# pierregab/VUB_Image_denoising

Measured on AMD Instinct MI355X. Metric: images/sec (256x256x3) RDUNet diffusion train step, higher is better.
Workload: dtype bf16; 1 GPU; RDUNet_T(base_filters=32) diffusion train step, fwd+Charbonnier+bwd+clip+AdamW; global_batch=16, per_gpu_batch=16, parallelism=dp1, optimizer_step=every step, launcher=single process

## Files before the change

### vub_image_denoising_amd/csrc/conv3_big.hip

```cpp
#include "conv3_tile.h"

#include <cstdlib>

namespace {

__device__ __attribute__((aligned(64))) unsigned int g_big_zero[16];


template <int N>
__device__ __forceinline__ void wait_vm() { asm volatile("s_waitcnt vmcnt(%0)" ::"n"(N) : "memory"); }

__device__ __forceinline__ void glds16(const void* src, unsigned dst) {
  unsigned keep;
  asm volatile("s_mov_b32 %0, m0\n\ts_mov_b32 m0, %2\n\ts_nop 0\n\tglobal_load_lds_dwordx4 %1, off\n\ts_mov_b32 m0, %0"
               : "=&s"(keep)
               : "v"(src), "s"(__builtin_amdgcn_readfirstlane(dst))
               : "memory");
}
__device__ __forceinline__ unsigned lds_addr(const unsigned char* p) {
  return (unsigned)(uintptr_t)(const __attribute__((address_space(3))) unsigned char*)p;
}

constexpr int TWB = 16;
constexpr int RS = TWB + 2;
constexpr int LDS_CAP = 160 * 1024;
constexpr int COL_MAX = 640;

enum { EP_FWD = 0, EP_FWD_RES = 1, EP_PLAIN = 2, EP_ACC = 3, EP_RES = 4 };

template <int CK>
__device__ __forceinline__ int hswz(int u, int x) {
  return CK == 64 ? (u ^ (x & 7)) : (u ^ ((x >> 1) & 3));
}

template <int TH, int BN, int WM, int CK, int NW = 8>
struct PtCfg {
  static constexpr int NTB = 64 * NW;
  static constexpr int BPC = NW == 8 ? 1 : 2;
  static constexpr int BM = TH * TWB;
  static constexpr int HWP = (TH + 2) * RS;
  static constexpr int RB = CK * 2;
  static constexpr int H_PIECES = (HWP * RB + 1023) / 1024;
  static constexpr int HALO_BYTES = H_PIECES * 1024;
  static constexpr int KC = (9 * CK + 63) / 64 * 64;
  static constexpr int SPC = KC / 64;
  static constexpr int SS = (SPC + 1) / 2;
  static constexpr int RW = 256;
  static constexpr int W_BYTES = BN * RW;
  static constexpr int W_PIECES = W_BYTES / 1024;
  static constexpr int W_PW = (W_PIECES + NW - 1) / NW;
  static constexpr int TAB = 2 * COL_MAX * 4;
  static constexpr int LDS = 2 * HALO_BYTES + 2 * W_BYTES + TAB;
  static constexpr int WN = NW / WM;
  static constexpr int WTM = BM / WM, WTN = BN / WN;
  static constexpr int MT = WTM / 16, NTL = WTN / 16;
  static constexpr bool OK = BPC * LDS <= LDS_CAP && MT >= 1 && NTL >= 1 && WTM % 16 == 0 && WTN % 16 == 0 &&
                             (CK == 32 || CK == 64) && WM * WN == NW && (NW == 8 || NW == 4);
};

template <int NLO, int NHI, int SPLIT>
__device__ __forceinline__ void wait_split(int wave) {
  if (wave < SPLIT) wait_vm<NHI>();
  else wait_vm<NLO>();
}

template <int TH, int BN, int WM, int CK, int EP, bool GO, int NW = 8>
__global__ __launch_bounds__(64 * NW, 2) void conv3_big_kernel(rdn_conv_desc d, int tiles_x, int tiles_y, int nitems) {
  using Cfg = PtCfg<TH, BN, WM, CK, NW>;
  constexpr int NTB = Cfg::NTB;
  constexpr int RB = Cfg::RB, RW = Cfg::RW, SPC = Cfg::SPC, SS = Cfg::SS;
  constexpr int WTN = Cfg::WTN, MT = Cfg::MT, NTL = Cfg::NTL, W_PW = Cfg::W_PW, HP = Cfg::H_PIECES;
  constexpr bool FWD = EP == EP_FWD || EP == EP_FWD_RES;
  constexpr bool RES = EP == EP_FWD_RES || EP == EP_RES;
  constexpr bool ACC = EP == EP_ACC;
  constexpr bool GOK = GO && !FWD;
  constexpr bool W16 = !GOK && MT % 2 == 0;
  static_assert(Cfg::OK, "conv3_big geometry");

  __shared__ __attribute__((aligned(1024))) unsigned char lds[Cfg::LDS];
  unsigned char* const halo = lds;
  unsigned char* const wst = lds + 2 * Cfg::HALO_BYTES;
  float* const tab = (float*)(wst + 2 * Cfg::W_BYTES);

  const int tid = threadIdx.x, lane = tid & 63, wave = tid >> 6;
  const int wm = wave % WM, wn = wave / WM;
  const int r = lane & 15, g = lane >> 4;
  const int ncb = d.ncols / BN;
  const int H = d.h, W = d.w;
  const int nch = d.cin / CK;

  const int per = gridDim.x >> 3, xcd = blockIdx.x & 7;
  const int it_lo = (int)((int64_t)nitems * xcd / 8), it_hi = (int)((int64_t)nitems * (xcd + 1) / 8);
  int item = it_lo + (blockIdx.x >> 3);

  const bool spre = (d.flags & RDN_EPI_STORE_PRE) != 0;
  if constexpr (FWD) {
    for (int c = tid; c < d.ncols; c += NTB) {
      tab[c] = d.bias[c];
      tab[COL_MAX + c] = d.alpha[c];
    }
  }
  if constexpr (GOK) {
    for (int c = tid; c < d.ncols - d.gout_c0; c += NTB) tab[COL_MAX + c] = d.gout_alpha[c];
  }

  struct Geo { int nimg, y0, x0, n0; };
  auto geo = [&](int itm) {
    Geo q;
    const int cb = itm % ncb;
    int t = itm / ncb;
    const int tx = t % tiles_x;
    t /= tiles_x;
    q.y0 = (t % tiles_y) * TH;
    q.x0 = tx * TWB;
    q.nimg = t / tiles_y;
    q.n0 = cb * BN;
    return q;
  };

  auto issue_h = [&](const Geo& q, int c, int hb) {
    const unsigned dst = lds_addr(halo) + hb * Cfg::HALO_BYTES;
    const bf16* const xb = (const bf16*)d.x + (((int64_t)q.nimg * H + (q.y0 - 1)) * W + (q.x0 - 1)) * d.x_ps;
#pragma unroll
    for (int k = 0; k < (HP + NW - 1) / NW; ++k) {
      const int pc = wave + NW * k;
      if (pc >= HP) break;
      const int off = pc * 1024 + lane * 16;
      const int hp = off / RB, pu = (off % RB) / 16;
      const int hy = hp / RS, hx = hp - (hp / RS) * RS;
      const int u = hswz<CK>(pu, hx);
      const bool ok =
          hp < Cfg::HWP && (unsigned)(q.y0 - 1 + hy) < (unsigned)H && (unsigned)(q.x0 - 1 + hx) < (unsigned)W;
      const void* src = ok ? (const void*)(xb + (int64_t)(hy * W + hx) * d.x_ps +
                                           rdn_coff32(d.x_c0 + c * CK + u * 8, (int)d.x_ps, (int)d.x_pl))
                           : (const void*)g_big_zero;
      glds16(src, dst + pc * 1024);
    }
  };
  auto issue_w = [&](int n0, int c, int jj, int wb) {
    const unsigned dst = lds_addr(wst) + wb * Cfg::W_BYTES;
#pragma unroll
    for (int k = 0; k < W_PW; ++k) {
      const int pc = wave + NW * k;
      if (pc >= Cfg::W_PIECES) break;
      const int row = 4 * pc + (lane >> 4);
      const int u = (lane & 15) ^ (row & 15);
      const bool ok = 2 * jj + 1 < SPC || u < 8;
      const void* src = ok ? (const void*)((const bf16*)d.wp + (int64_t)(n0 + row) * d.kp + c * Cfg::KC + jj * 128 +
                                           u * 8)
                           : (const void*)g_big_zero;
      glds16(src, dst + pc * 1024);
    }
  };

  int a_off[CK == 64 ? 6 : 3];
#pragma unroll
  for (int ks = 0; ks < (CK == 64 ? 2 : 1); ++ks)
#pragma unroll
    for (int dx = 0; dx < 3; ++dx) a_off[ks * 3 + dx] = (r + dx) * RB + hswz<CK>(ks * 4 + g, r + dx) * 16;
  const int a_row0 = (wm * MT) * RS * RB;
  const int b_lane = (wn * WTN + r) * RW;
  int b_off[4];
#pragma unroll
  for (int hk = 0; hk < 4; ++hk) b_off[hk] = ((hk * 4 + g) ^ r) * 16;

  f32x4 acc[MT][NTL];
  auto zero_acc = [&]() {
#pragma unroll
    for (int i = 0; i < MT; ++i)
#pragma unroll
      for (int jn = 0; jn < NTL; ++jn) acc[i][jn] = f32x4{0.f, 0.f, 0.f, 0.f};
  };

  auto compute_pf = [&](int jj, const unsigned char* ph, const unsigned char* pbs) {
    auto valid = [&](int q) { return 2 * jj + (q >> 1) < SPC && (2 * jj + (q >> 1)) * 64 + (q & 1) * 32 < 9 * CK; };
    u32x4 af[2][MT], bfr[2][NTL];
    auto rd = [&](int q, int buf) {
#ifdef BIG_DIAG_NO_LDS
#pragma unroll
      for (int i = 0; i < MT; ++i) asm volatile("" : "=v"(af[buf][i]));
#pragma unroll
      for (int jn = 0; jn < NTL; ++jn) asm volatile("" : "=v"(bfr[buf][jn]));
      return;
#endif
      const int k0 = (2 * jj + (q >> 1)) * 64 + (q & 1) * 32;
      const int tap = k0 / CK, ksub = (k0 - tap * CK) / 32;
      const int dy = tap / 3, dx = tap % 3;
      const unsigned char* pa = ph + a_row0 + dy * RS * RB + a_off[ksub * 3 + dx];
#pragma unroll
      for (int i = 0; i < MT; ++i) af[buf][i] = *(const u32x4*)(pa + i * RS * RB);
#pragma unroll
      for (int jn = 0; jn < NTL; ++jn) bfr[buf][jn] = *(const u32x4*)(pbs + jn * 16 * RW + b_off[q]);
    };
    rd(0, 0);
#pragma unroll
    for (int q = 0; q < 4; ++q) {
      if (!valid(q)) break;
      if (q + 1 < 4 && valid(q + 1)) rd(q + 1, (q + 1) & 1);
      __builtin_amdgcn_sched_barrier(0);
#ifdef BIG_DIAG_NO_MFMA
#pragma unroll
      for (int i = 0; i < MT; ++i) asm volatile("" ::"v"(af[q & 1][i]));
#pragma unroll
      for (int jn = 0; jn < NTL; ++jn) asm volatile("" ::"v"(bfr[q & 1][jn]));
      continue;
#endif
#pragma unroll
      for (int i = 0; i < MT; ++i)
#pragma unroll
        for (int jn = 0; jn < NTL; ++jn)
          acc[i][jn] = __builtin_amdgcn_mfma_f32_16x16x32_bf16(__builtin_bit_cast(bf16x8, bfr[q & 1][jn]),
                                                               __builtin_bit_cast(bf16x8, af[q & 1][i]), acc[i][jn], 0,
                                                               0, 0);
    }
  };
  auto compute_roll = [&](int jj, const unsigned char* ph, const unsigned char* pbs) {
    auto valid = [&](int q) { return 2 * jj + (q >> 1) < SPC && (2 * jj + (q >> 1)) * 64 + (q & 1) * 32 < 9 * CK; };
    u32x4 af[MT], bfr[2][NTL];
    auto pa_of = [&](int q) {
      const int k0 = (2 * jj + (q >> 1)) * 64 + (q & 1) * 32;
      const int tap = k0 / CK, ksub = (k0 - tap * CK) / 32;
      const int dy = tap / 3, dx = tap % 3;
      return ph + a_row0 + dy * RS * RB + a_off[ksub * 3 + dx];
    };
    auto rdb = [&](int q, int buf) {
#pragma unroll
      for (int jn = 0; jn < NTL; ++jn) bfr[buf][jn] = *(const u32x4*)(pbs + jn * 16 * RW + b_off[q]);
    };
    {
      const unsigned char* pa = pa_of(0);
#pragma unroll
      for (int i = 0; i < MT; ++i) af[i] = *(const u32x4*)(pa + i * RS * RB);
      rdb(0, 0);
    }
#pragma unroll
    for (int q = 0; q < 4; ++q) {
      if (!valid(q)) break;
      const bool nx = q + 1 < 4 && valid(q + 1);
      if (nx) rdb(q + 1, (q + 1) & 1);
      const unsigned char* pn = pa_of(nx ? q + 1 : q);
#pragma unroll
      for (int i = 0; i < MT; ++i) {
        __builtin_amdgcn_sched_barrier(0);
#pragma unroll
        for (int jn = 0; jn < NTL; ++jn)
          acc[i][jn] = __builtin_amdgcn_mfma_f32_16x16x32_bf16(__builtin_bit_cast(bf16x8, bfr[q & 1][jn]),
                                                               __builtin_bit_cast(bf16x8, af[i]), acc[i][jn], 0, 0, 0);
        __builtin_amdgcn_sched_barrier(0);
        if (nx) af[i] = *(const u32x4*)(pn + i * RS * RB);
      }
    }
  };
  auto compute_np = [&](int jj, const unsigned char* ph, const unsigned char* pbs) {
#pragma unroll
    for (int h = 0; h < 2; ++h) {
      const int j = 2 * jj + h;
      if (j >= SPC) break;
#pragma unroll
      for (int ks = 0; ks < 2; ++ks) {
        const int k0 = j * 64 + ks * 32;
        if (k0 >= 9 * CK) break;
        const int tap = k0 / CK, ksub = (k0 - tap * CK) / 32;
        const int dy = tap / 3, dx = tap % 3;
        const unsigned char* pa = ph + a_row0 + dy * RS * RB + a_off[ksub * 3 + dx];
        __builtin_amdgcn_sched_barrier(0);
        u32x4 af[MT], bfr[NTL];
#pragma unroll
        for (int i = 0; i < MT; ++i) af[i] = *(const u32x4*)(pa + i * RS * RB);
#pragma unroll
        for (int jn = 0; jn < NTL; ++jn) bfr[jn] = *(const u32x4*)(pbs + jn * 16 * RW + b_off[2 * h + ks]);
#pragma unroll
        for (int i = 0; i < MT; ++i)
#pragma unroll
          for (int jn = 0; jn < NTL; ++jn)
            acc[i][jn] = __builtin_amdgcn_mfma_f32_16x16x32_bf16(__builtin_bit_cast(bf16x8, bfr[jn]),
                                                                 __builtin_bit_cast(bf16x8, af[i]), acc[i][jn], 0, 0,
                                                                 0);
      }
    }
  };
  constexpr bool ROLL = BN == 128 && CK == 64 && (GOK || EP == EP_FWD_RES);
  constexpr bool NOPF = BN == 128 && CK == 64 && GOK && EP == EP_RES;
  auto compute = [&](int jj, const unsigned char* ph, const unsigned char* pbs) {
    if constexpr (NOPF) compute_np(jj, ph, pbs);
    else if constexpr (ROLL) compute_roll(jj, ph, pbs);
    else compute_pf(jj, ph, pbs);
  };

  u32x2 eop[(RES || ACC) ? MT : 1][(RES || ACC) ? NTL : 1];
  u32x2 gpre[GOK ? MT : 1][GOK ? NTL : 1];
  auto epi_load = [&](const Geo& q) {
    const int64_t pix0 = ((int64_t)q.nimg * H + q.y0) * W + q.x0;
    const bool col_ok = q.x0 + r < W;
    if constexpr ((RES || ACC) && W16) {
      const int ops = (int)d.out_ps;
      const int eps = RES ? (int)d.res_ps : ops;
      const __amdgpu_buffer_rsrc_t re =
          rdn_rsrc(RES ? (const bf16*)d.res + pix0 * d.res_ps : (const bf16*)d.out + pix0 * d.out_ps);
#pragma unroll
      for (int jn = 0; jn < NTL; ++jn) {
        const int cl = q.n0 + wn * WTN + jn * 16 + 8 * (g >> 1);
        const int coff =
            RES ? rdn_coff32(d.res_c0 + cl, eps, (int)d.res_pl) : rdn_coff32(d.out_c0 + cl, ops, (int)d.out_pl);
        const bool cok = col_ok & (RES ? cl < d.res_climit : true);
#pragma unroll
        for (int p = 0; p < MT / 2; ++p) {
          const int i = 2 * p + (g & 1);
          const bool ok = cok & (q.y0 + wm * MT + i < H);
          const u32x4 u = rdn_ld16(re, ok, (((wm * MT + i) * W + r) * eps + coff) * 2);
          eop[2 * p][jn] = u32x2{u[0], u[1]};
          eop[2 * p + 1][jn] = u32x2{u[2], u[3]};
        }
      }
    } else if constexpr (RES || ACC) {
      const int ops = (int)d.out_ps;
      const int eps = RES ? (int)d.res_ps : ops;
      const __amdgpu_buffer_rsrc_t re =
          rdn_rsrc(RES ? (const bf16*)d.res + pix0 * d.res_ps : (const bf16*)d.out + pix0 * d.out_ps);
#pragma unroll
      for (int jn = 0; jn < NTL; ++jn) {
        const int cl = q.n0 + wn * WTN + jn * 16 + g * 4;
        const int coff =
            RES ? rdn_coff32(d.res_c0 + cl, eps, (int)d.res_pl) : rdn_coff32(d.out_c0 + cl, ops, (int)d.out_pl);
        const bool cok = col_ok & (RES ? cl < d.res_climit : true);
#pragma unroll
        for (int i = 0; i < MT; ++i) {
          const bool ok = cok & (q.y0 + wm * MT + i < H);
          eop[i][jn] = rdn_ld8(re, ok, (((wm * MT + i) * W + r) * eps + coff) * 2);
        }
      }
    }
    if constexpr (GOK) {
      const __amdgpu_buffer_rsrc_t rg = rdn_rsrc((const bf16*)d.gout_pre + pix0 * d.gout_pre_ps);
      const int gps = (int)d.gout_pre_ps;
#pragma unroll
      for (int jn = 0; jn < NTL; ++jn) {
        const int cl = q.n0 + wn * WTN + jn * 16 + g * 4;
        const bool gok = col_ok & (cl >= d.gout_c0);
#pragma unroll
        for (int i = 0; i < MT; ++i)
          gpre[i][jn] = rdn_ld8(rg, gok & (q.y0 + wm * MT + i < H), (((wm * MT + i) * W + r) * gps + cl - d.gout_c0) * 2);
      }
    }
  };
  auto epilogue16 = [&](const Geo& q) {
    epi_load(q);
    const int64_t pix0 = ((int64_t)q.nimg * H + q.y0) * W + q.x0;
    const __amdgpu_buffer_rsrc_t ro = rdn_rsrc((const bf16*)d.out + pix0 * d.out_ps);
    const int ops = (int)d.out_ps, pps = (int)d.pre_ps;
    const bool col_ok = q.x0 + r < W;
    const __amdgpu_buffer_rsrc_t rp = FWD && spre ? rdn_rsrc((const bf16*)d.pre + pix0 * d.pre_ps) : ro;
#pragma unroll
    for (int jn = 0; jn < NTL; ++jn) {
      const int cl = q.n0 + wn * WTN + jn * 16 + 8 * (g >> 1);
      f32x4 b0 = {0.f, 0.f, 0.f, 0.f}, b1 = b0, a0 = b0, a1 = b0;
      if constexpr (FWD) {
        b0 = *(const f32x4*)(tab + cl);
        b1 = *(const f32x4*)(tab + cl + 4);
        a0 = *(const f32x4*)(tab + COL_MAX + cl);
        a1 = *(const f32x4*)(tab + COL_MAX + cl + 4);
      }
      const int co = rdn_coff32(d.out_c0 + cl, ops, (int)d.out_pl);
      const int cp = FWD ? rdn_coff32(cl, pps, (int)d.pre_pl) : 0;
      const bool res_ok = RES ? cl < d.res_climit : true;
#pragma unroll
      for (int p = 0; p < MT / 2; ++p) {
        const int i = 2 * p + (g & 1);
        const bool ok = col_ok & (q.y0 + wm * MT + i < H);
        const int prow = (wm * MT + i) * W + r;
        const u32x4 ua = __builtin_bit_cast(u32x4, acc[2 * p][jn]), ub = __builtin_bit_cast(u32x4, acc[2 * p + 1][jn]);
        u32x4 lo, hi;
#pragma unroll
        for (int e = 0; e < 4; ++e) {
          const auto sw = __builtin_amdgcn_permlane16_swap(ua[e], ub[e], false, false);
          lo[e] = sw[0];
          hi[e] = sw[1];
        }
        const f32x4 flo = __builtin_bit_cast(f32x4, lo), fhi = __builtin_bit_cast(f32x4, hi);
        float v[8];
#pragma unroll
        for (int e = 0; e < 4; ++e) {
          v[e] = flo[e];
          v[4 + e] = fhi[e];
        }
        if constexpr (FWD) {
#pragma unroll
          for (int e = 0; e < 4; ++e) {
            v[e] += b0[e];
            v[4 + e] += b1[e];
          }
          int o = ok && spre ? (prow * pps + cp) * 2 : RDN_OOB;
          asm volatile("" : "+v"(o));
          __builtin_amdgcn_raw_buffer_store_b128(__builtin_bit_cast(u32x4, Unit16<bf16>::pack(v)), rp, o, 0, 0);
#pragma unroll
          for (int e = 0; e < 4; ++e) {
            v[e] = v[e] > 0.f ? v[e] : a0[e] * v[e];
            v[4 + e] = v[4 + e] > 0.f ? v[4 + e] : a1[e] * v[4 + e];
          }
        }
        if constexpr (RES || ACC) {
          if (res_ok) {
            v[0] += bf16lo(eop[2 * p][jn][0]); v[1] += bf16hi(eop[2 * p][jn][0]);
            v[2] += bf16lo(eop[2 * p][jn][1]); v[3] += bf16hi(eop[2 * p][jn][1]);
            v[4] += bf16lo(eop[2 * p + 1][jn][0]); v[5] += bf16hi(eop[2 * p + 1][jn][0]);
            v[6] += bf16lo(eop[2 * p + 1][jn][1]); v[7] += bf16hi(eop[2 * p + 1][jn][1]);
          }
        }
        int o = ok ? (prow * ops + co) * 2 : RDN_OOB;
        asm volatile("" : "+v"(o));
        __builtin_amdgcn_raw_buffer_store_b128(__builtin_bit_cast(u32x4, Unit16<bf16>::pack(v)), ro, o, 0, 0);
      }
    }
  };
  auto epilogue = [&](const Geo& q, int itm) {
    if constexpr (W16) {
      (void)itm;
      epilogue16(q);
      return;
    }
    epi_load(q);
    const int64_t pix0 = ((int64_t)q.nimg * H + q.y0) * W + q.x0;
    const __amdgpu_buffer_rsrc_t ro = rdn_rsrc((const bf16*)d.out + pix0 * d.out_ps);
    const __amdgpu_buffer_rsrc_t rgo = GOK ? rdn_rsrc((const bf16*)d.gout + pix0 * d.gout_ps) : ro;
    const int ops = (int)d.out_ps, pps = (int)d.pre_ps;
    const bool col_ok = q.x0 + r < W;
    const __amdgpu_buffer_rsrc_t rp = FWD && spre ? rdn_rsrc((const bf16*)d.pre + pix0 * d.pre_ps) : ro;
#pragma unroll
    for (int jn = 0; jn < NTL; ++jn) {
      const int cl = q.n0 + wn * WTN + jn * 16 + g * 4;
      f32x4 bias = {0.f, 0.f, 0.f, 0.f}, alpha = {0.f, 0.f, 0.f, 0.f};
      if constexpr (FWD) {
        bias = *(const f32x4*)(tab + cl);
        alpha = *(const f32x4*)(tab + COL_MAX + cl);
      }
      const int co = rdn_coff32(d.out_c0 + cl, ops, (int)d.out_pl);
      const int cp = FWD ? rdn_coff32(cl, pps, (int)d.pre_pl) : 0;
      const bool res_ok = RES ? cl < d.res_climit : true;
      float gsa[4] = {0.f, 0.f, 0.f, 0.f}, gsb[4] = {0.f, 0.f, 0.f, 0.f};
#pragma unroll
      for (int i = 0; i < MT; ++i) {
        const bool ok = col_ok & (q.y0 + wm * MT + i < H);
        const int prow = (wm * MT + i) * W + r;
        float v[4] = {acc[i][jn][0], acc[i][jn][1], acc[i][jn][2], acc[i][jn][3]};
        if constexpr (FWD) {
#pragma unroll
          for (int e = 0; e < 4; ++e) v[e] += bias[e];
          int o = ok && spre ? (prow * pps + cp) * 2 : RDN_OOB;
          asm volatile("" : "+v"(o));
          __builtin_amdgcn_raw_buffer_store_b64(rdn_pack4(v), rp, o, 0, 0);
#pragma unroll
          for (int e = 0; e < 4; ++e) v[e] = v[e] > 0.f ? v[e] : alpha[e] * v[e];
        }
        if constexpr (RES || ACC) {
          if (res_ok) {
            v[0] += bf16lo(eop[i][jn][0]); v[1] += bf16hi(eop[i][jn][0]);
            v[2] += bf16lo(eop[i][jn][1]); v[3] += bf16hi(eop[i][jn][1]);
          }
        }
        if constexpr (GOK) {
          if (cl >= d.gout_c0) {
            const int gc = cl - d.gout_c0;
            const f32x4 al = *(const f32x4*)(tab + COL_MAX + gc);
            const float pr[4] = {bf16lo(gpre[i][jn][0]), bf16hi(gpre[i][jn][0]), bf16lo(gpre[i][jn][1]),
                                 bf16hi(gpre[i][jn][1])};
#pragma unroll
            for (int e = 0; e < 4; ++e) {
              const bool pos = pr[e] > 0.f;
              if (ok && !pos) gsa[e] += pr[e] * v[e];
              v[e] = pos ? v[e] : al[e] * v[e];
              if (ok) gsb[e] += v[e];
            }
            int o = ok ? (prow * (int)d.gout_ps + gc) * 2 : RDN_OOB;
            asm volatile("" : "+v"(o));
            __builtin_amdgcn_raw_buffer_store_b64(rdn_pack4(v), rgo, o, 0, 0);
            continue;
          }
        }
        int o = ok ? (prow * ops + co) * 2 : RDN_OOB;
        asm volatile("" : "+v"(o));
        __builtin_amdgcn_raw_buffer_store_b64(rdn_pack4(v), ro, o, 0, 0);
      }
      if constexpr (GOK) {
        if (cl >= d.gout_c0) {
#pragma unroll
          for (int e = 0; e < 4; ++e)
#pragma unroll
            for (int m = 1; m < 16; m <<= 1) {
              gsa[e] += __shfl_xor(gsa[e], m, 64);
              gsb[e] += __shfl_xor(gsb[e], m, 64);
            }
          if (r == 0) {
            const int gcn = d.ncols - d.gout_c0;
            float* const prt = d.gout_part + ((int64_t)(itm / ncb) * WM + wm) * 2 * gcn + (cl - d.gout_c0);
            *(f32x4*)prt = f32x4{gsa[0], gsa[1], gsa[2], gsa[3]};
            *(f32x4*)(prt + gcn) = f32x4{gsb[0], gsb[1], gsb[2], gsb[3]};
          }
        }
      }
    }
  };

  Geo cur = geo(item < it_hi ? item : it_lo);
  if (item < it_hi) {
    issue_w(cur.n0, 0, 0, 0);
    issue_h(cur, 0, 0);
  }
  wait_vm<0>();
  __syncthreads();
  int wbuf = 0, hbuf = 0;
  while (item < it_hi) {
    const int nxt_item = item + per;
    const bool has_next = nxt_item < it_hi;
    const Geo nq = geo(has_next ? nxt_item : item);
    zero_acc();
    for (int c = 0; c < nch; ++c) {
      const bool more = c + 1 < nch;
      const unsigned char* const ph = halo + hbuf * Cfg::HALO_BYTES;
#pragma unroll
      for (int jj = 0; jj < SS; ++jj) {
        const bool nxt = jj + 1 < SS || more || has_next;
#ifdef BIG_DIAG_NO_DMA
        if (false) {
#else
        if (nxt) {
#endif
          if (jj + 1 < SS) issue_w(cur.n0, c, jj + 1, wbuf ^ 1);
          else if (more) issue_w(cur.n0, c + 1, 0, wbuf ^ 1);
          else issue_w(nq.n0, 0, 0, wbuf ^ 1);
        }
#ifdef BIG_DIAG_NO_DMA
        const bool hl = false;
#else
        const bool hl = jj == 0 && (more || has_next);
#endif
        if (hl) issue_h(more ? cur : nq, more ? c + 1 : 0, hbuf ^ 1);
        compute(jj, ph, wst + wbuf * Cfg::W_BYTES + b_lane);
#ifndef BIG_DIAG_NO_BAR
        if (hl && SS > 1) wait_split<HP / NW, HP / NW + 1, HP % NW>(wave);
        else wait_vm<0>();
        __builtin_amdgcn_s_barrier();
#endif
        asm volatile("" ::: "memory");
        wbuf ^= 1;
      }
      hbuf ^= 1;
    }
#ifdef BIG_DIAG_NO_EPI
    {
      float t = 0.f;
#pragma unroll
      for (int i = 0; i < MT; ++i)
#pragma unroll
        for (int jn = 0; jn < NTL; ++jn) t += acc[i][jn][0] + acc[i][jn][3];
      if (t == 1.2345f) ((float*)d.out)[tid] = t;
    }
#else
    epilogue(cur, item);
#endif
    item = nxt_item;
    cur = nq;
  }
}

int big_mode() {
  static const int m = [] {
    const char* e = getenv("RDN_BIG");
    return (e && e[0] == '0') ? 0 : 1;
  }();
  return m;
}

int cu_count() {
  static int cus = 0;
  if (!cus) {
    int dev = 0, n = 0;
    (void)hipGetDevice(&dev);
    if (hipDeviceGetAttribute(&n, hipDeviceAttributeMultiprocessorCount, dev) != hipSuccess || n < 8) n = 256;
    cus = n;
  }
  return cus;
}

int epi_mode(const rdn_conv_desc* d) {
  const int f = d->flags & ~RDN_EPI_STORE_PRE;
  const int fwd = RDN_EPI_BIAS | RDN_EPI_PRELU;
  if (f == fwd) return EP_FWD;
  if (f == (fwd | RDN_EPI_RESID)) return EP_FWD_RES;
  if (d->flags & RDN_EPI_STORE_PRE) return -1;
  if (f == 0) return EP_PLAIN;
  if (f == RDN_EPI_ACCUM) return EP_ACC;
  if (f == RDN_EPI_RESID) return EP_RES;
  return -1;
}

template <int TH, int BN, int WM, int CK, int EP, bool GO = false, int NW = 8>
int launch_pt(const rdn_conv_desc* d, hipStream_t st, int tiles_x, int tiles_y, int nitems) {
  using Cfg = PtCfg<TH, BN, WM, CK, NW>;
  if constexpr (!Cfg::OK) {
    return 1;
  } else {
    constexpr bool FWD_ = EP == EP_FWD || EP == EP_FWD_RES;
    if constexpr (!(GO && !FWD_) && Cfg::MT % 2 == 0) {
      auto a8 = [](int64_t ps, int64_t c0, const void* p) { return ps % 8 == 0 && c0 % 8 == 0 && !((uintptr_t)p & 15); };
      if (!a8(d->out_ps, d->out_c0, d->out)) return 1;
      if (FWD_ && !a8(d->pre_ps, 0, d->pre)) return 1;
      if ((EP == EP_FWD_RES || EP == EP_RES) && (!a8(d->res_ps, d->res_c0, d->res) || d->res_climit % 8)) return 1;
    }
    if (GO) rdn_probe_rows = (int)((int64_t)d->n * tiles_x * tiles_y * WM);
    RDN_PROBE("conv3_big_kernel<bf16,%d,%d,%d,%d%s%s>", TH, BN, WM, CK, GO ? ",go" : "", NW == 4 ? ",w4" : "");
    const int per_xcd = (nitems + 7) / 8;
    int slots = Cfg::BPC * cu_count() / 8;
    if (slots > per_xcd) slots = per_xcd;
    if (slots < 1) slots = 1;
    hipLaunchKernelGGL((conv3_big_kernel<TH, BN, WM, CK, EP, GO, NW>), dim3((unsigned)(8 * slots)), dim3(Cfg::NTB), 0,
                       st, *d, tiles_x, tiles_y, nitems);
    return rdn_check_launch("rdn_conv_fwd(conv3 big)");
  }
}

template <int TH, int BN, int WM, int CK, int NW = 8>
int launch_big(const rdn_conv_desc* d, hipStream_t st) {
  const int tiles_x = (d->w + TWB - 1) / TWB, tiles_y = (d->h + TH - 1) / TH;
  const int64_t nitems = (int64_t)d->n * tiles_x * tiles_y * (d->ncols / BN);
  if (nitems >= (1ll << 31)) return 1;
  const int ni = (int)nitems;
  if (d->gout) {
    if constexpr (NW == 8) {
      switch (epi_mode(d)) {
        case EP_PLAIN: return launch_pt<TH, BN, WM, CK, EP_PLAIN, true>(d, st, tiles_x, tiles_y, ni);
        case EP_ACC: return launch_pt<TH, BN, WM, CK, EP_ACC, true>(d, st, tiles_x, tiles_y, ni);
        case EP_RES: return launch_pt<TH, BN, WM, CK, EP_RES, true>(d, st, tiles_x, tiles_y, ni);
      }
    }
    return 1;
  }
  switch (epi_mode(d)) {
    case EP_FWD: return launch_pt<TH, BN, WM, CK, EP_FWD, false, NW>(d, st, tiles_x, tiles_y, ni);
    case EP_FWD_RES: return launch_pt<TH, BN, WM, CK, EP_FWD_RES, false, NW>(d, st, tiles_x, tiles_y, ni);
    case EP_PLAIN: return launch_pt<TH, BN, WM, CK, EP_PLAIN, false, NW>(d, st, tiles_x, tiles_y, ni);
    case EP_ACC: return launch_pt<TH, BN, WM, CK, EP_ACC, false, NW>(d, st, tiles_x, tiles_y, ni);
    case EP_RES: return launch_pt<TH, BN, WM, CK, EP_RES, false, NW>(d, st, tiles_x, tiles_y, ni);
  }
  return 1;
}

bool big_ck32_multi() {
  static const bool on = [] {
    const char* e = getenv("RDN_BIG_CK32");
    return !(e && e[0] == '0');
  }();
  return on;
}

bool big_nw4() {
  static const bool on = [] {
    const char* e = getenv("RDN_BIG_NW4");
    return !(e && e[0] == '0');
  }();
  return on;
}

bool big_fall() {
  static const bool on = [] {
    const char* e = getenv("RDN_BIG_FALL");
    return !(e && e[0] == '0');
  }();
  return on;
}

template <int CK>
int big_dispatch(const rdn_conv_desc* d, hipStream_t st) {
  const int64_t tiles = (int64_t)d->n * ((d->h + 15) / 16) * ((d->w + 15) / 16);
  const int cus = cu_count(), nch = d->cin / CK;
  if (CK == 32 && nch != 1 && !big_ck32_multi()) return 1;
  auto even = [&](int64_t items) {
    const int64_t rounds = (items + cus - 1) / cus;
    return items >= cus && items * 10 >= rounds * cus * 9;
  };
  const bool big_img = (int64_t)d->h * d->w >= 128 * 128;
  static const bool loose = [] {
    const char* e = getenv("RDN_BIG_LOOSE");
    return !(e && e[0] == '0');
  }();
  auto wide_ok = [&](int bn) {
    const int64_t items = tiles * (d->ncols / bn);
    return even(items) && ((loose && bn == 128) || nch >= 2 || (items >= 4ll * cus && big_img));
  };
  auto narrow_ok = [&](int bn) {
    const int64_t items = tiles * (d->ncols / bn);
    return even(items) && ((loose && bn == 64) || (items * nch >= 8ll * cus && big_img));
  };
  if (d->ncols % 128 == 0) return wide_ok(128) ? launch_big<16, 128, 4, CK>(d, st) : 1;
  if (d->ncols % 96 == 0) return wide_ok(96) ? launch_big<16, 96, 4, CK>(d, st) : 1;
  if (d->ncols % 80 == 0) {
    if (narrow_ok(80)) return launch_big<16, 80, 8, CK>(d, st);
    if (!(big_fall() && d->ncols % 64 == 0 && tiles * (d->ncols / 64) <= 6ll * cus)) return 1;
  }
  if (d->ncols % 64 == 0) {
    if (!narrow_ok(64)) return 1;
    if constexpr (CK == 32)
      if (big_nw4() && !d->gout) return launch_big<16, 64, 4, CK, 4>(d, st);
    return launch_big<16, 64, 4, CK>(d, st);
  }
  if (d->ncols == 32) {
    if constexpr (CK == 64) {
      const int64_t items = tiles;
      return (even(items) && items >= 4ll * cus && big_img) ? launch_big<16, 32, 8, CK>(d, st) : 1;
    }
  }
  return 1;
}

}

int rdn_conv3_big_launch(const rdn_conv_desc* d, int ck, hipStream_t st) {
  if (!big_mode() || d->dtype != RDN_BF16 || d->gather != RDN_G_CONV3) return 1;
  if (d->bn || d->bm || d->gate) return 1;
  if (ck != 32 && ck != 64) return 1;
  if (epi_mode(d) < 0) return 1;
  if (d->ncols % 16 || d->ncols < 32 || d->cin < 32 || d->ncols > COL_MAX) return 1;
  if (d->x_ps % 8 || d->x_c0 % 8 || ((uintptr_t)d->x & 15) || ((uintptr_t)d->wp & 15) || d->kp % 8) return 1;
  if (d->out_ps % 4 || d->out_c0 % 4 || ((uintptr_t)d->out & 7)) return 1;
  if ((d->flags & RDN_EPI_STORE_PRE) && (d->pre_ps % 4 || ((uintptr_t)d->pre & 7))) return 1;
  if ((d->flags & RDN_EPI_RESID) && (d->res_ps % 4 || d->res_c0 % 4 || d->res_climit % 4 || ((uintptr_t)d->res & 7)))
    return 1;
  const int64_t px = (int64_t)d->n * d->h * d->w;
  if (px < 8192) return 1;
  auto fits = [&](int64_t ps, int64_t pl, int c_hi) {
    return 2 * ((int64_t)(18 + 1) * d->w * ps + rdn_coff(c_hi, ps, pl)) < (int64_t)RDN_OOB - 16;
  };
  if (!fits(d->x_ps, d->x_pl, d->x_c0 + d->cin) || !fits(d->out_ps, d->out_pl, d->out_c0 + d->ncols) ||
      ((d->flags & RDN_EPI_STORE_PRE) && !fits(d->pre_ps, d->pre_pl, d->ncols)) ||
      ((d->flags & RDN_EPI_RESID) && !fits(d->res_ps, d->res_pl, d->res_c0 + d->res_climit)))
    return 1;
  if (d->gout && (d->ncols - d->gout_c0 > COL_MAX || d->gout_c0 % 4 || d->gout_ps % 4 || d->gout_pre_ps % 4 ||
                  !fits(d->gout_ps, 0, d->ncols - d->gout_c0) || !fits(d->gout_pre_ps, 0, d->ncols - d->gout_c0) ||
                  ((uintptr_t)d->gout_part & 15)))
    return 1;
  return ck == 64 ? big_dispatch<64>(d, st) : big_dispatch<32>(d, st);
}
```

### vub_image_denoising_amd/csrc/conv3_halo.hip

```cpp
#include "conv3_tile.h"

#include <cstdlib>

namespace {

constexpr int NT = 256;
using c3::TH;
using c3::TW;
using c3::BM;
using c3::HW_;
using c3::HaloRow;
constexpr int ROWB = 160;

template <typename T, int BN, int WMW, int CK, bool GATE, bool PAIR_OK, bool SPLIT = false>
__global__ __launch_bounds__(NT, (BN >= 64 ? 1 : 2)) void conv3_halo_kernel(rdn_conv_desc d, int tiles_x, int tiles_y,
                                                                          int c_per = 0, float* __restrict__ ws = nullptr) {
  constexpr int ES = sizeof(T);
  constexpr int VEC = TypeInfo<T>::VEC;
  constexpr int SK = 128 / ES;
  constexpr int KSTEP = 4 * VEC;
  constexpr int CKB = CK * ES;
  constexpr int HROW = HaloRow<CKB>::V;
  constexpr int SPC = (9 * CK + SK - 1) / SK;
  constexpr int KC = SPC * SK;
// ... 441 lines not shown
}

constexpr int MIN_BLOCKS = 512;

static int pick_bn(int ncols, int64_t tiles) {
  int bn = pick_bn_cols(ncols);
  while ((bn == 128 || bn == 64) && ncols % (bn / 2) == 0 &&
         tiles * ((ncols + bn - 1) / bn) < (int64_t)MIN_BLOCKS)
    bn /= 2;
  return bn;
}

template <typename T, int CK>
int launch_bn(const rdn_conv_desc* d, hipStream_t st, int splits = 0, float* ws = nullptr) {
  const int64_t tiles = (int64_t)d->n * ((d->h + c3::TH - 1) / c3::TH) * ((d->w + c3::TW - 1) / c3::TW);
  const int bn = d->bn ? d->bn : pick_bn(d->ncols, tiles);
  switch (bn) {
    case 16: return launch_h<T, 16, 4, CK>(d, st, splits, ws);
    case 32: return launch_h<T, 32, 4, CK>(d, st, splits, ws);
    case 48: return launch_h<T, 48, 4, CK>(d, st, splits, ws);
    case 64: return launch_h<T, 64, 2, CK>(d, st, splits, ws);
    case 80: return launch_h<T, 80, 4, CK>(d, st, splits, ws);
    case 96: return launch_h<T, 96, 4, CK>(d, st, splits, ws);
    case 128: return launch_h<T, 128, 2, CK>(d, st, splits, ws);
  }
  rdn_set_error("rdn_conv_fwd(conv3): unsupported bn=%d", bn);
  return RDN_E_ARG;
}

}

int rdn_conv3_chunk_pow2(int cin, int cap) {
  int ck = cap;
  while (ck > 8 && (cin % ck)) ck >>= 1;
  return (cin % ck) ? -1 : ck;
}

int rdn_conv3_chunk_impl(int cin, int dtype) {
  if (dtype == RDN_BF16 && (cin == 48 || cin == 80 || cin == 96)) return cin;
  return rdn_conv3_chunk_pow2(cin, dtype == RDN_BF16 ? 64 : 32);
}

extern "C" int rdn_conv3_chunk(int32_t cin, int32_t dtype) { return rdn_conv3_chunk_impl(cin, dtype); }

extern "C" int rdn_conv3_packed_k(int32_t cin, int32_t dtype) {
  const int ck = rdn_conv3_chunk_impl(cin, dtype);
  if (ck < 0) return RDN_E_SHAPE;
  const int sk = dtype == RDN_BF16 ? 64 : 32;
  const int kc = (9 * ck + sk - 1) / sk * sk;
  const int kp = (cin / ck) * kc;
  return (kp + 63) / 64 * 64;
}

extern "C" int rdn_conv3_pick_bn(int32_t ncols) { return pick_bn_cols(ncols); }

int rdn_conv3_launch(const rdn_conv_desc* d, hipStream_t st) {
  const int ck = rdn_conv3_chunk_impl(d->cin, d->dtype);
  if (d->gate && (!d->gate_alpha || d->gate_ps % (d->dtype == RDN_BF16 ? 8 : 4) || ((uintptr_t)d->gate & 15))) {
    rdn_set_error("rdn_conv_fwd(conv3): gate needs alpha and 16-byte aligned rows"); return RDN_E_ARG;
  }
  if (ck < 0) { rdn_set_error("rdn_conv_fwd(conv3): cin=%d not a multiple of 8", d->cin); return RDN_E_SHAPE; }
  if (d->kp < rdn_conv3_packed_k(d->cin, d->dtype)) {
    rdn_set_error("rdn_conv_fwd(conv3): kp=%d < packed K %d (pack with ck=%d)", d->kp,
                  rdn_conv3_packed_k(d->cin, d->dtype), ck);
    return RDN_E_SHAPE;
  }
  if (d->dtype == RDN_BF16) {
    const int big = rdn_conv3_big_launch(d, ck, st);
    if (big <= 0) return big;
    const int wsd = rdn_conv3_wsd_launch(d, ck, st);
    if (wsd <= 0) return wsd;
    const int ws = rdn_conv3_ws_launch(d, ck, st);
    if (ws <= 0) return ws;
    switch (ck) {
      case 96: return launch_bn<bf16, 96>(d, st);
      case 80: return launch_bn<bf16, 80>(d, st);
      case 48: return launch_bn<bf16, 48>(d, st);
      case 64: return launch_bn<bf16, 64>(d, st);
      case 32: return launch_bn<bf16, 32>(d, st);
      case 16: return launch_bn<bf16, 16>(d, st);
      default: return launch_bn<bf16, 8>(d, st);
    }
  }
  switch (ck) {
    case 32: return launch_bn<float, 32>(d, st);
    case 16: return launch_bn<float, 16>(d, st);
    default: return launch_bn<float, 8>(d, st);
  }
}

int rdn_conv3_splitk_slices(const rdn_conv_desc* d, int cus) {
  if (d->gather != RDN_G_CONV3 || d->gate || d->gout || (d->flags & RDN_EPI_SCATTER2) || d->ncols % 4) return 0;
  const int ck = rdn_conv3_chunk_impl(d->cin, d->dtype);
  if (ck <= 0) return 0;
  const int nch = d->cin / ck;
  const int64_t tiles = (int64_t)d->n * ((d->h + c3::TH - 1) / c3::TH) * ((d->w + c3::TW - 1) / c3::TW);
  const int bn = d->bn ? d->bn : pick_bn(d->ncols, tiles);
  const int64_t base = tiles * ((d->ncols + bn - 1) / bn);
  if (nch < 2 || 2 * base > cus) return 0;
  int s = (int)((rdn_splitk_target(cus) + base - 1) / base);
  if (s > nch) s = nch;
  const int c_per = (nch + s - 1) / s;
  return (nch + c_per - 1) / c_per;
}

int rdn_conv3_splitk_launch(const rdn_conv_desc* d, int splits, float* ws, hipStream_t st) {
  const int ck = rdn_conv3_chunk_impl(d->cin, d->dtype);
  if (d->dtype == RDN_BF16) {
    switch (ck) {
      case 96: return launch_bn<bf16, 96>(d, st, splits, ws);
      case 80: return launch_bn<bf16, 80>(d, st, splits, ws);
      case 48: return launch_bn<bf16, 48>(d, st, splits, ws);
      case 64: return launch_bn<bf16, 64>(d, st, splits, ws);
      case 32: return launch_bn<bf16, 32>(d, st, splits, ws);
      case 16: return launch_bn<bf16, 16>(d, st, splits, ws);
      default: return launch_bn<bf16, 8>(d, st, splits, ws);
    }
  }
  switch (ck) {
    case 32: return launch_bn<float, 32>(d, st, splits, ws);
    case 16: return launch_bn<float, 16>(d, st, splits, ws);
    default: return launch_bn<float, 8>(d, st, splits, ws);
  }
}
```

Baseline: 1886 images/s.

## Add 8-row, 4-wave conv3 big-tile variant for small spatial layers

Adds an 8x16-pixel, 4-wave, 64-channel-chunk configuration of the big conv3 kernel. It is routed to for low-resolution layers (at most 64x64) with specific cin/ncols shapes, and is reached when the existing big dispatch declines. The variant includes an interleaved row-ownership mode for gate-out backward, which has its own epilogue that reduces partial sums across waves through LDS. It also shrinks the bias/slope table to free LDS, and adds an explicit bm=128 entry path with error messages. The aim is better occupancy and tile fit on small deep layers that previously fell to halo or other kernels. The cost is more code paths and hardcoded shape tables.

```diff
diff --git a/vub_image_denoising_amd/csrc/conv3_big.hip b/vub_image_denoising_amd/csrc/conv3_big.hip
--- a/vub_image_denoising_amd/csrc/conv3_big.hip
+++ b/vub_image_denoising_amd/csrc/conv3_big.hip
@@ -49,11 +49,13 @@
   static constexpr int W_BYTES = BN * RW;
   static constexpr int W_PIECES = W_BYTES / 1024;
   static constexpr int W_PW = (W_PIECES + NW - 1) / NW;
-  static constexpr int TAB = 2 * COL_MAX * 4;
+  static constexpr int COLT = (NW == 4 && CK == 64) ? 256 : COL_MAX;
+  static constexpr int TAB = 2 * COLT * 4;
   static constexpr int LDS = 2 * HALO_BYTES + 2 * W_BYTES + TAB;
   static constexpr int WN = NW / WM;
   static constexpr int WTM = BM / WM, WTN = BN / WN;
   static constexpr int MT = WTM / 16, NTL = WTN / 16;
+  static constexpr bool HORD = TH == 8 && WM == 2 && NW == 4;
   static constexpr bool OK = BPC * LDS <= LDS_CAP && MT >= 1 && NTL >= 1 && WTM % 16 == 0 && WTN % 16 == 0 &&
                              (CK == 32 || CK == 64) && WM * WN == NW && (NW == 8 || NW == 4);
 };
@@ -70,6 +72,7 @@
   constexpr int NTB = Cfg::NTB;
   constexpr int RB = Cfg::RB, RW = Cfg::RW, SPC = Cfg::SPC, SS = Cfg::SS;
   constexpr int WTN = Cfg::WTN, MT = Cfg::MT, NTL = Cfg::NTL, W_PW = Cfg::W_PW, HP = Cfg::H_PIECES;
+  constexpr int COLT = Cfg::COLT;
   constexpr bool FWD = EP == EP_FWD || EP == EP_FWD_RES;
   constexpr bool RES = EP == EP_FWD_RES || EP == EP_RES;
   constexpr bool ACC = EP == EP_ACC;
@@ -85,6 +88,8 @@
   const int tid = threadIdx.x, lane = tid & 63, wave = tid >> 6;
   const int wm = wave % WM, wn = wave / WM;
   const int r = lane & 15, g = lane >> 4;
+  constexpr bool HORD = Cfg::HORD && GOK;
+  constexpr int RSTEP = HORD ? WM : 1;
   const int ncb = d.ncols / BN;
   const int H = d.h, W = d.w;
   const int nch = d.cin / CK;
@@ -97,11 +102,11 @@
   if constexpr (FWD) {
     for (int c = tid; c < d.ncols; c += NTB) {
       tab[c] = d.bias[c];
-      tab[COL_MAX + c] = d.alpha[c];
+      tab[COLT + c] = d.alpha[c];
     }
   }
   if constexpr (GOK) {
-    for (int c = tid; c < d.ncols - d.gout_c0; c += NTB) tab[COL_MAX + c] = d.gout_alpha[c];
+    for (int c = tid; c < d.ncols - d.gout_c0; c += NTB) tab[COLT + c] = d.gout_alpha[c];
   }
 
   struct Geo { int nimg, y0, x0, n0; };
@@ -158,7 +163,7 @@
   for (int ks = 0; ks < (CK == 64 ? 2 : 1); ++ks)
 #pragma unroll
     for (int dx = 0; dx < 3; ++dx) a_off[ks * 3 + dx] = (r + dx) * RB + hswz<CK>(ks * 4 + g, r + dx) * 16;
-  const int a_row0 = (wm * MT) * RS * RB;
+  const int a_row0 = (HORD ? wm : wm * MT) * RS * RB;
   const int b_lane = (wn * WTN + r) * RW;
   int b_off[4];
 #pragma unroll
@@ -188,7 +193,7 @@
       const int dy = tap / 3, dx = tap % 3;
       const unsigned char* pa = ph + a_row0 + dy * RS * RB + a_off[ksub * 3 + dx];
 #pragma unroll
-      for (int i = 0; i < MT; ++i) af[buf][i] = *(const u32x4*)(pa + i * RS * RB);
+      for (int i = 0; i < MT; ++i) af[buf][i] = *(const u32x4*)(pa + i * RSTEP * RS * RB);
 #pragma unroll
       for (int jn = 0; jn < NTL; ++jn) bfr[buf][jn] = *(const u32x4*)(pbs + jn * 16 * RW + b_off[q]);
     };
@@ -230,7 +235,7 @@
     {
       const unsigned char* pa = pa_of(0);
 #pragma unroll
-      for (int i = 0; i < MT; ++i) af[i] = *(const u32x4*)(pa + i * RS * RB);
+      for (int i = 0; i < MT; ++i) af[i] = *(const u32x4*)(pa + i * RSTEP * RS * RB);
       rdb(0, 0);
     }
 #pragma unroll
@@ -247,7 +252,7 @@
           acc[i][jn] = __builtin_amdgcn_mfma_f32_16x16x32_bf16(__builtin_bit_cast(bf16x8, bfr[q & 1][jn]),
                                                                __builtin_bit_cast(bf16x8, af[i]), acc[i][jn], 0, 0, 0);
         __builtin_amdgcn_sched_barrier(0);
-        if (nx) af[i] = *(const u32x4*)(pn + i * RS * RB);
+        if (nx) af[i] = *(const u32x4*)(pn + i * RSTEP * RS * RB);
       }
     }
   };
@@ -266,7 +271,7 @@
         __builtin_amdgcn_sched_barrier(0);
         u32x4 af[MT], bfr[NTL];
 #pragma unroll
-        for (int i = 0; i < MT; ++i) af[i] = *(const u32x4*)(pa + i * RS * RB);
+        for (int i = 0; i < MT; ++i) af[i] = *(const u32x4*)(pa + i * RSTEP * RS * RB);
 #pragma unroll
         for (int jn = 0; jn < NTL; ++jn) bfr[jn] = *(const u32x4*)(pbs + jn * 16 * RW + b_off[2 * h + ks]);
 #pragma unroll
@@ -357,8 +362,8 @@
       if constexpr (FWD) {
         b0 = *(const f32x4*)(tab + cl);
         b1 = *(const f32x4*)(tab + cl + 4);
-        a0 = *(const f32x4*)(tab + COL_MAX + cl);
-        a1 = *(const f32x4*)(tab + COL_MAX + cl + 4);
+        a0 = *(const f32x4*)(tab + COLT + cl);
+        a1 = *(const f32x4*)(tab + COLT + cl + 4);
       }
       const int co = rdn_coff32(d.out_c0 + cl, ops, (int)d.out_pl);
       const int cp = FWD ? rdn_coff32(cl, pps, (int)d.pre_pl) : 0;
@@ -431,7 +436,7 @@
       f32x4 bias = {0.f, 0.f, 0.f, 0.f}, alpha = {0.f, 0.f, 0.f, 0.f};
       if constexpr (FWD) {
         bias = *(const f32x4*)(tab + cl);
-        alpha = *(const f32x4*)(tab + COL_MAX + cl);
+        alpha = *(const f32x4*)(tab + COLT + cl);
       }
       const int co = rdn_coff32(d.out_c0 + cl, ops, (int)d.out_pl);
       const int cp = FWD ? rdn_coff32(cl, pps, (int)d.pre_pl) : 0;
@@ -460,7 +465,7 @@
         if constexpr (GOK) {
           if (cl >= d.gout_c0) {
             const int gc = cl - d.gout_c0;
-            const f32x4 al = *(const f32x4*)(tab + COL_MAX + gc);
+            const f32x4 al = *(const f32x4*)(tab + COLT + gc);
             const float pr[4] = {bf16lo(gpre[i][jn][0]), bf16hi(gpre[i][jn][0]), bf16lo(gpre[i][jn][1]),
                                  bf16hi(gpre[i][jn][1])};
 #pragma unroll
@@ -495,6 +500,122 @@
             *(f32x4*)prt = f32x4{gsa[0], gsa[1], gsa[2], gsa[3]};
             *(f32x4*)(prt + gcn) = f32x4{gsb[0], gsb[1], gsb[2], gsb[3]};
           }
+        }
+      }
+    }
+  };
+  auto epilogue_hord = [&](const Geo& q, int itm) {
+    const int64_t pix0 = ((int64_t)q.nimg * H + q.y0) * W + q.x0;
+    const __amdgpu_buffer_rsrc_t ro = rdn_rsrc((const bf16*)d.out + pix0 * d.out_ps);
+    const __amdgpu_buffer_rsrc_t rgo = rdn_rsrc((const bf16*)d.gout + pix0 * d.gout_ps);
+    const __amdgpu_buffer_rsrc_t rg = rdn_rsrc((const bf16*)d.gout_pre + pix0 * d.gout_pre_ps);
+    const int ops = (int)d.out_ps, gps = (int)d.gout_pre_ps;
+    const bool col_ok = q.x0 + r < W;
+    u32x2 eo[(RES || ACC) ? MT : 1][(RES || ACC) ? NTL : 1], gp[MT][NTL];
+    if constexpr (RES || ACC) {
+      const int eps = RES ? (int)d.res_ps : ops;
+      const __amdgpu_buffer_rsrc_t re =
+          rdn_rsrc(RES ? (const bf16*)d.res + pix0 * d.res_ps : (const bf16*)d.out + pix0 * d.out_ps);
+#pragma unroll
+      for (int jn = 0; jn < NTL; ++jn) {
+        const int cl = q.n0 + wn * WTN + jn * 16 + g * 4;
+        const int coff =
+            RES ? rdn_coff32(d.res_c0 + cl, eps, (int)d.res_pl) : rdn_coff32(d.out_c0 + cl, ops, (int)d.out_pl);
+        const bool cok = col_ok & (RES ? cl < d.res_climit : true);
+#pragma unroll
+        for (int i = 0; i < MT; ++i) {
+          const int row = wm + i * WM;
+          eo[i][jn] = rdn_ld8(re, cok & (q.y0 + row < H), ((row * W + r) * eps + coff) * 2);
+        }
+      }
+    }
+#pragma unroll
+    for (int jn = 0; jn < NTL; ++jn) {
+      const int cl = q.n0 + wn * WTN + jn * 16 + g * 4;
+      const bool gok = col_ok & (cl >= d.gout_c0);
+#pragma unroll
+      for (int i = 0; i < MT; ++i) {
+        const int row = wm + i * WM;
+        gp[i][jn] = rdn_ld8(rg, gok & (q.y0 + row < H), ((row * W + r) * gps + cl - d.gout_c0) * 2);
+      }
+    }
+    f32x4 hsa[NTL], hsb[NTL];
+#pragma unroll
+    for (int jn = 0; jn < NTL; ++jn) {
+      const int cl = q.n0 + wn * WTN + jn * 16 + g * 4;
+      const int co = rdn_coff32(d.out_c0 + cl, ops, (int)d.out_pl);
+      const bool res_ok = RES ? cl < d.res_climit : true;
+      const bool gated = cl >= d.gout_c0;
+      const int gc = cl - d.gout_c0;
+      f32x4 al = {0.f, 0.f, 0.f, 0.f};
+      if (gated) al = *(const f32x4*)(tab + COLT + gc);
+      float gsa[4] = {0.f, 0.f, 0.f, 0.f}, gsb[4] = {0.f, 0.f, 0.f, 0.f};
+#pragma unroll
+      for (int i = 0; i < MT; ++i) {
+        const int row = wm + i * WM;
+        const bool ok = col_ok & (q.y0 + row < H);
+        const int prow = row * W + r;
+        float v[4] = {acc[i][jn][0], acc[i][jn][1], acc[i][jn][2], acc[i][jn][3]};
+        if constexpr (RES || ACC) {
+          if (res_ok) {
+            v[0] += bf16lo(eo[i][jn][0]); v[1] += bf16hi(eo[i][jn][0]);
+            v[2] += bf16lo(eo[i][jn][1]); v[3] += bf16hi(eo[i][jn][1]);
+          }
+        }
+        if (gated) {
+          const float pr[4] = {bf16lo(gp[i][jn][0]), bf16hi(gp[i][jn][0]), bf16lo(gp[i][jn][1]), bf16hi(gp[i][jn][1])};
+#pragma unroll
+          for (int e = 0; e < 4; ++e) {
+            const bool pos = pr[e] > 0.f;
+            if (ok && !pos) gsa[e] = __builtin_fmaf(pr[e], v[e], gsa[e]);
+            v[e] = pos ? v[e] : al[e] * v[e];
+            if (ok) gsb[e] += v[e];
+          }
+          int o = ok ? (prow * (int)d.gout_ps + gc) * 2 : RDN_OOB;
+          asm volatile("" : "+v"(o));
+          __builtin_amdgcn_raw_buffer_store_b64(rdn_pack4(v), rgo, o, 0, 0);
+          continue;
+        }
+        int o = ok ? (prow * ops + co) * 2 : RDN_OOB;
+        asm volatile("" : "+v"(o));
+        __builtin_amdgcn_raw_buffer_store_b64(rdn_pack4(v), ro, o, 0, 0);
+      }
+      if (gated) {
+#pragma unroll
+        for (int e = 0; e < 4; ++e)
+#pragma unroll
+          for (int m = 1; m < 16; m <<= 1) {
+            gsa[e] += __shfl_xor(gsa[e], m, 64);
+            gsb[e] += __shfl_xor(gsb[e], m, 64);
+          }
+      }
+      hsa[jn] = f32x4{gsa[0], gsa[1], gsa[2], gsa[3]};
+      hsb[jn] = f32x4{gsb[0], gsb[1], gsb[2], gsb[3]};
+    }
+    float* const xch = tab;
+    if (wm == 1 && r == 0) {
+#pragma unroll
+      for (int jn = 0; jn < NTL; ++jn) {
+        const int lc = wn * WTN + jn * 16 + g * 4;
+        if (q.n0 + lc >= d.gout_c0) {
+          *(f32x4*)(xch + lc) = hsa[jn];
+          *(f32x4*)(xch + BN + lc) = hsb[jn];
+        }
+      }
+    }
+    asm volatile("s_waitcnt lgkmcnt(0)" ::: "memory");
+    __builtin_amdgcn_s_barrier();
+    asm volatile("" ::: "memory");
+    if (wm == 0 && r == 0) {
+      const int gcn = d.ncols - d.gout_c0;
+#pragma unroll
+      for (int jn = 0; jn < NTL; ++jn) {
+        const int lc = wn * WTN + jn * 16 + g * 4, cl = q.n0 + lc;
+        if (cl >= d.gout_c0) {
+          const f32x4 oa = *(const f32x4*)(xch + lc), ob = *(const f32x4*)(xch + BN + lc);
+          float* const prt = d.gout_part + (int64_t)(itm / ncb) * 2 * gcn + (cl - d.gout_c0);
+          *(f32x4*)prt = hsa[jn] + oa;
+          *(f32x4*)(prt + gcn) = hsb[jn] + ob;
         }
       }
     }
@@ -555,7 +676,8 @@
       if (t == 1.2345f) ((float*)d.out)[tid] = t;
     }
 #else
-    epilogue(cur, item);
+    if constexpr (HORD) epilogue_hord(cur, item);
+    else epilogue(cur, item);
 #endif
     item = nxt_item;
     cur = nq;
@@ -600,13 +722,15 @@
     return 1;
   } else {
     constexpr bool FWD_ = EP == EP_FWD || EP == EP_FWD_RES;
+    if (FWD_ && d->ncols > Cfg::COLT) return 1;
+    if (GO && d->ncols - d->gout_c0 > Cfg::COLT) return 1;
     if constexpr (!(GO && !FWD_) && Cfg::MT % 2 == 0) {
       auto a8 = [](int64_t ps, int64_t c0, const void* p) { return ps % 8 == 0 && c0 % 8 == 0 && !((uintptr_t)p & 15); };
       if (!a8(d->out_ps, d->out_c0, d->out)) return 1;
       if (FWD_ && !a8(d->pre_ps, 0, d->pre)) return 1;
       if ((EP == EP_FWD_RES || EP == EP_RES) && (!a8(d->res_ps, d->res_c0, d->res) || d->res_climit % 8)) return 1;
     }
-    if (GO) rdn_probe_rows = (int)((int64_t)d->n * tiles_x * tiles_y * WM);
+    if (GO) rdn_probe_rows = (int)((int64_t)d->n * tiles_x * tiles_y * (Cfg::HORD ? 1 : WM));
     RDN_PROBE("conv3_big_kernel<bf16,%d,%d,%d,%d%s%s>", TH, BN, WM, CK, GO ? ",go" : "", NW == 4 ? ",w4" : "");
     const int per_xcd = (nitems + 7) / 8;
     int slots = Cfg::BPC * cu_count() / 8;
@@ -625,11 +749,11 @@
   if (nitems >= (1ll << 31)) return 1;
   const int ni = (int)nitems;
   if (d->gout) {
-    if constexpr (NW == 8) {
+    if constexpr (NW == 8 || TH == 8) {
       switch (epi_mode(d)) {
-        case EP_PLAIN: return launch_pt<TH, BN, WM, CK, EP_PLAIN, true>(d, st, tiles_x, tiles_y, ni);
-        case EP_ACC: return launch_pt<TH, BN, WM, CK, EP_ACC, true>(d, st, tiles_x, tiles_y, ni);
-        case EP_RES: return launch_pt<TH, BN, WM, CK, EP_RES, true>(d, st, tiles_x, tiles_y, ni);
+        case EP_PLAIN: return launch_pt<TH, BN, WM, CK, EP_PLAIN, true, NW>(d, st, tiles_x, tiles_y, ni);
+        case EP_ACC: return launch_pt<TH, BN, WM, CK, EP_ACC, true, NW>(d, st, tiles_x, tiles_y, ni);
+        case EP_RES: return launch_pt<TH, BN, WM, CK, EP_RES, true, NW>(d, st, tiles_x, tiles_y, ni);
       }
     }
     return 1;
@@ -711,31 +835,108 @@
   return 1;
 }
 
-}
-
-int rdn_conv3_big_launch(const rdn_conv_desc* d, int ck, hipStream_t st) {
-  if (!big_mode() || d->dtype != RDN_BF16 || d->gather != RDN_G_CONV3) return 1;
-  if (d->bn || d->bm || d->gate) return 1;
-  if (ck != 32 && ck != 64) return 1;
-  if (epi_mode(d) < 0) return 1;
-  if (d->ncols % 16 || d->ncols < 32 || d->cin < 32 || d->ncols > COL_MAX) return 1;
-  if (d->x_ps % 8 || d->x_c0 % 8 || ((uintptr_t)d->x & 15) || ((uintptr_t)d->wp & 15) || d->kp % 8) return 1;
-  if (d->out_ps % 4 || d->out_c0 % 4 || ((uintptr_t)d->out & 7)) return 1;
-  if ((d->flags & RDN_EPI_STORE_PRE) && (d->pre_ps % 4 || ((uintptr_t)d->pre & 7))) return 1;
+
+int big_t8_mode() {
+  static const int m = [] {
+    const char* e = getenv("RDN_BIG_T8");
+    return !e ? 1 : e[0] == '0' ? 0 : e[0] == '2' ? 2 : 1;
+  }();
+  return m;
+}
+
+int big_t8_wm_env() {
+  const char* e = getenv("RDN_BIG_T8_WM");
+  return e && (e[0] == '2' || e[0] == '4') && !e[1] ? e[0] - '0' : 0;
+}
+
+int launch_t8(const rdn_conv_desc* d, hipStream_t st, int wm) {
+  return wm == 4 ? launch_big<8, 64, 4, 64, 4>(d, st) : launch_big<8, 64, 2, 64, 4>(d, st);
+}
+
+const char* big_pre(const rdn_conv_desc* d, int ck, int halo_rows) {
+  if (d->dtype != RDN_BF16 || d->gather != RDN_G_CONV3) return "bf16 3x3 convs only";
+  if (d->gate) return "gated inputs are not served (conv3_halo)";
+  if (ck != 32 && ck != 64) return "needs 32- or 64-channel chunks";
+  if (epi_mode(d) < 0) return "epilogue flags not served";
+  if (d->ncols % 16 || d->ncols < 32 || d->cin < 32 || d->ncols > COL_MAX) return "ncols / cin out of range";
+  if (d->x_ps % 8 || d->x_c0 % 8 || ((uintptr_t)d->x & 15) || ((uintptr_t)d->wp & 15) || d->kp % 8)
+    return "input / weight alignment";
+  if (d->out_ps % 4 || d->out_c0 % 4 || ((uintptr_t)d->out & 7)) return "output alignment";
+  if ((d->flags & RDN_EPI_STORE_PRE) && (d->pre_ps % 4 || ((uintptr_t)d->pre & 7))) return "pre alignment";
   if ((d->flags & RDN_EPI_RESID) && (d->res_ps % 4 || d->res_c0 % 4 || d->res_climit % 4 || ((uintptr_t)d->res & 7)))
-    return 1;
-  const int64_t px = (int64_t)d->n * d->h * d->w;
-  if (px < 8192) return 1;
+    return "residual alignment";
   auto fits = [&](int64_t ps, int64_t pl, int c_hi) {
-    return 2 * ((int64_t)(18 + 1) * d->w * ps + rdn_coff(c_hi, ps, pl)) < (int64_t)RDN_OOB - 16;
+    return 2 * ((int64_t)(halo_rows + 1) * d->w * ps + rdn_coff(c_hi, ps, pl)) < (int64_t)RDN_OOB - 16;
   };
   if (!fits(d->x_ps, d->x_pl, d->x_c0 + d->cin) || !fits(d->out_ps, d->out_pl, d->out_c0 + d->ncols) ||
       ((d->flags & RDN_EPI_STORE_PRE) && !fits(d->pre_ps, d->pre_pl, d->ncols)) ||
       ((d->flags & RDN_EPI_RESID) && !fits(d->res_ps, d->res_pl, d->res_c0 + d->res_climit)))
-    return 1;
+    return "an item's offsets pass 32 bits";
   if (d->gout && (d->ncols - d->gout_c0 > COL_MAX || d->gout_c0 % 4 || d->gout_ps % 4 || d->gout_pre_ps % 4 ||
                   !fits(d->gout_ps, 0, d->ncols - d->gout_c0) || !fits(d->gout_pre_ps, 0, d->ncols - d->gout_c0) ||
                   ((uintptr_t)d->gout_part & 15)))
-    return 1;
-  return ck == 64 ? big_dispatch<64>(d, st) : big_dispatch<32>(d, st);
-}
+    return "gate-out operands";
+  return nullptr;
+}
+
+const char* t8_pre(const rdn_conv_desc* d, int ck) {
+  if (ck != 64) return "needs 64-channel chunks (cin % 64 == 0)";
+  if (d->ncols % 64) return "needs ncols % 64 == 0";
+  using Cfg = PtCfg<8, 64, 2, 64, 4>;
+  const int ep = epi_mode(d);
+  if ((ep == EP_FWD || ep == EP_FWD_RES) && d->ncols > Cfg::COLT) return "forward ncols past the bias / slope table";
+  if (d->gout && d->ncols - d->gout_c0 > Cfg::COLT) return "gated columns past the slope table";
+  if (d->gout && (d->h % 8 || d->w % TWB)) return "gate-out needs full 8x16 tiles";
+  return nullptr;
+}
+
+int big_t8_wm(const rdn_conv_desc* d) {
+  if ((int64_t)d->h * d->w > 64 * 64) return 0;
+  const int ep = epi_mode(d), k = d->cin, n = d->ncols;
+  if (ep == EP_FWD || ep == EP_FWD_RES)
+    return (k == 640 && n == 256) || ((k == 256 || k == 384 || k == 512) && n == 128) ? 2 : 0;
+  return (k == 64 && n == 192) || (k == 128 && (n == 320 || n == 256)) || (k == 256 && n == 640) ? 2 : 0;
+}
+
+int t8_dispatch(const rdn_conv_desc* d, hipStream_t st) {
+  const int mode = big_t8_mode();
+  if (!mode || t8_pre(d, 64)) return 1;
+  int wm = big_t8_wm_env();
+  if (mode != 2) {
+    const int64_t items = (int64_t)d->n * ((d->h + 7) / 8) * ((d->w + 15) / 16) * (d->ncols / 64);
+    if (items < 2ll * cu_count()) return 1;
+    const int lw = big_t8_wm(d);
+    if (!lw) return 1;
+    if (!wm) wm = lw;
+  }
+  return launch_t8(d, st, wm ? wm : 2);
+}
+
+}
+
+int rdn_conv3_big_launch(const rdn_conv_desc* d, int ck, hipStream_t st) {
+  if (d->bm == 128 && !d->bn) {
+    const char* why = big_pre(d, ck, 10);
+    if (!why) why = t8_pre(d, ck);
+    if (!why && (int64_t)d->n * d->h * d->w < 8192) why = "fewer than 8192 pixels";
+    if (why) {
+      rdn_set_error("rdn_conv_fwd(conv3 big, bm=128): %s", why);
+      return RDN_E_SHAPE;
+    }
+    const int wm = big_t8_wm_env();
+    const int rc = launch_t8(d, st, wm ? wm : big_t8_wm(d) ? big_t8_wm(d) : 2);
+    if (rc == 1) {
+      rdn_set_error("rdn_conv_fwd(conv3 big, bm=128): operands not 8-channel aligned for the 16-byte epilogue");
+      return RDN_E_SHAPE;
+    }
+    return rc;
+  }
+  if (!big_mode() || d->bn || d->bm) return 1;
+  const int64_t px = (int64_t)d->n * d->h * d->w;
+  if (px >= 8192 && !big_pre(d, ck, 18)) {
+    const int rc = ck == 64 ? big_dispatch<64>(d, st) : big_dispatch<32>(d, st);
+    if (rc != 1) return rc;
+  }
+  if (ck != 64 || (px < 8192 && big_t8_mode() != 2) || big_pre(d, ck, 10)) return 1;
+  return t8_dispatch(d, st);
+}
diff --git a/vub_image_denoising_amd/csrc/conv3_halo.hip b/vub_image_denoising_amd/csrc/conv3_halo.hip
--- a/vub_image_denoising_amd/csrc/conv3_halo.hip
+++ b/vub_image_denoising_amd/csrc/conv3_halo.hip
@@ -547,6 +547,10 @@
       default: return launch_bn<bf16, 8>(d, st);
     }
   }
+  if (d->bm == 128 && !d->bn) {
+    rdn_set_error("rdn_conv_fwd(conv3 big, bm=128): bf16 only");
+    return RDN_E_SHAPE;
+  }
   switch (ck) {
     case 32: return launch_bn<float, 32>(d, st);
     case 16: return launch_bn<float, 16>(d, st);
```

Result: no change. 1902 images/s, median of 6 (+0.9%).
